# ChicyChen/LOCO-Edit

Measured on AMD Instinct MI355X. Metric: edit-directions/sec (top-5 PMP-Jacobian SVD @256^2) + vT cos-sim vs ref, higher is better.
Workload: dtype bf16x3 (split-bf16 MFMA operands, fp32 accumulate + fp32 storage); 1 GPU; CelebA-HQ DDPM 256x256 top-5 local basis (l_eye-sized mask, L=2400), t=0.6T, 12 power iterations, one GPU; multi_gpu_form=single, probes_total=5, probes_per_gpu=5, kept=5, n_iter=12, mask_L=2400, weights=synthetic seed 0, streams=2

## Files before the change

### include/loco_hip_diag.h

```cpp
#ifndef LOCO_HIP_DIAG_H
#define LOCO_HIP_DIAG_H
#include "loco_hip.h"
#ifdef __cplusplus
extern "C" {
#endif

int  loco_bench_conv(loco_ctx* ctx, int32_t cin, int32_t cout, int32_t H, int32_t W, int32_t B, int32_t mode,
                     int32_t taps, int32_t tile, int32_t iters, float* ms_avg, void* stream);

typedef struct loco_conv_desc {
    int32_t struct_size;
    int32_t Cin, Cout, Hin, Win, B, taps;
    int32_t stride, upsample, zins, mode, cpg;
    int32_t transposed, accumulate, in_arena, pad;
    int32_t Cin2, cot_cpg;
    float   res_scale;
    int32_t st_cpg;
    const float *weight, *bias;
    const float *in, *bias2, *res;
    const float *prim, *sc, *sh, *mr, *gamma, *tst, *tc;
    const float *in2, *w2, *bias2nd;
    const float *cot_d, *cot_prim, *cot_sc, *cot_sh, *cot_mr, *cot_tc;
    float* out;
    const float *st_prim, *st_mr;
// ... 59 lines not shown
    int32_t op, kind, act, B, C, T, H, W, n, k, accumulate, cos_first;
    float   eps, scale, t, cv, ce;
    float   f[5];
    int32_t pad_;
    int64_t count, split, in_bs, out_bs, aux_bs, st_bs;
    const float *x, *y, *stats, *gamma, *beta, *base;
    const float *freq, *w0, *b0, *w1, *b1, *add, *add_in;
    const float *src[4];
    const uint8_t *mask, *mask2;
    float *out, *out2, *t_dev;
} loco_pointwise_desc;
int  loco_debug_pointwise(loco_ctx* ctx, const loco_pointwise_desc* desc, void* stream);

int64_t loco_debug_tensor(loco_ctx* ctx, const char* name, float* dst, int64_t cap, void* stream);

#ifdef __cplusplus
}
#endif
#endif
```

### loco-edit_amd/csrc/conv_bf16_kernel.h

```cpp
#pragma once
#include "kernels.h"
#include <cstdlib>
#include <type_traits>

namespace loco {


typedef float f32x16 __attribute__((ext_vector_type(16)));
typedef float f32x4 __attribute__((ext_vector_type(4)));
typedef f32x4 f32x4_u __attribute__((aligned(4)));
typedef float f32x2 __attribute__((ext_vector_type(2)));
typedef f32x2 f32x2_u __attribute__((aligned(4)));
typedef __bf16 bf16x8 __attribute__((ext_vector_type(8)));
typedef _Float16 f16x8 __attribute__((ext_vector_type(8)));
typedef short s16x8 __attribute__((ext_vector_type(8)));

enum : int { PR_BF16X3 = 0, PR_F16 = 1 };

constexpr int BKC = 16;
constexpr bool LIVE_MASK = true;
constexpr bool EARLY_W = true;
constexpr int NDUMMY = 8;

__device__ __forceinline__ float sigmoidf2_(float y) { return __builtin_amdgcn_rcpf(1.0f + __expf(-y)); }
// ... 507 lines not shown
        }
        tile_id = __builtin_amdgcn_readfirstlane(tile_id);
        cot_id = __builtin_amdgcn_readfirstlane(cot_id);
        zid = __builtin_amdgcn_readfirstlane(zid);
    }
    int ty0_, tx0_;
    idivmod_small(tile_id, tiles_x, ty0_, tx0_);
    const int oy0 = __builtin_amdgcn_readfirstlane(ty0_ * TH);
    const int ox0 = __builtin_amdgcn_readfirstlane(tx0_ * TW);
    const int co0 = cot_id * MT;
    int zb_, zs_;
    idivmod_small(zid, a.nsplit, zb_, zs_);
    const int b = __builtin_amdgcn_readfirstlane(zb_);
    const int split = __builtin_amdgcn_readfirstlane(zs_);

    if constexpr (XPF && PHASE != 2 && EARLY_W) {
        const int nchunks_ = (a.Cin + BKC - 1) / BKC;
        const int cps_ = __builtin_amdgcn_readfirstlane((nchunks_ + a.nsplit - 1) / a.nsplit);
        const int cbeg_ = split * cps_;
        const int cend_ = (cbeg_ + cps_ < nchunks_) ? cbeg_ + cps_ : nchunks_;
        if (cend_ > cbeg_) {
            typedef __attribute__((address_space(3))) unsigned char lds_u8_;
            typedef const __attribute__((address_space(1))) unsigned char glb_u8_;
            const int wpitch_ = (a.Cout + 31) & ~31;
            const unsigned char* wbase0 = reinterpret_cast<const unsigned char*>(a.wb) +
                                          (unsigned)(cbeg_ * TAPS) * ((unsigned)wpitch_ * (unsigned)RB);
#pragma unroll
            for (int st_ = 0; st_ < 2; ++st_)
#pragma unroll
                for (int i = 0; i < NWV; ++i) {
// ... 837 lines not shown
```

### loco-edit_amd/csrc/conv_plan.hip

```cpp
#include "kernels.h"
#include <cstdio>
#include <cstdlib>

namespace loco {

constexpr int BKC = 16;
constexpr int BKF = 8;

static const int kMT[6] = {128, 128, 32, 64, 128, 128}, kNT[6] = {128, 64, 128, 64, 256, 256};

static int env_int(const char* name, int dflt) {
    const char* e = getenv(name);
    return e ? atoi(e) : dflt;
}
static int pick_tile(int Cout, int HW) {
    if (HW >= 128) return Cout > 32 ? 0 : 2;
    return Cout > 64 ? 1 : 3;
}

static int conv_pick_nsplit(int Cin, int Cout, int Hout, int Wout, int B) {
    const int t = pick_tile(Cout, Hout * Wout);
    long blocks = (long)((Hout * Wout) / kNT[t]) * ((Cout + kMT[t] - 1) / kMT[t]) * B;
    int nchunks = (Cin + BKF - 1) / BKF;
    if (blocks >= 384 || nchunks < 8) return 1;
// ... 14 lines not shown
    return t;
}

constexpr int kTile0MaxHW = 65536;

static int bf16_tile_of(const ConvArgs& a, int tile_override = -1) {
    int tile = conv_bf16_pick_tile(a.Cout, a.Hout * a.Wout, a.B, tile_override);
    if (tile == 4) tile = 5;
    if (tile == 5 && a.taps == 1 && !a.gemm && a.B >= 2 && a.Hout * a.Wout <= kTile0MaxHW) return 0;
    if (a.stride == 2 && tile == 5) tile = 0;
    return tile;
}
static int tile_for(const ConvArgs& a, int prec, int tile_override) {
    return prec ? bf16_tile_of(a, tile_override) : pick_tile(a.Cout, a.Hout * a.Wout);
}
static int conv_bf16_tile_pixels(const ConvArgs& a) { return a.poly == 1 ? 512 : a.gemm ? 256 : kNT[a.tile]; }
int conv_bf16_tile_couts(const ConvArgs& a) { return a.gemm ? 64 * a.gemm_tm : kMT[a.tile]; }

static bool conv_poly_ok(const ConvEnv& e, const ConvArgs& a, int taps) {
    static const bool on = env_int("LOCO_POLYPHASE", 1) != 0;
    if (!on || e.prec < 1 || taps != 9 || a.mode != CM_NONE || !(a.upsample || a.zins) || a.stride != 1) return false;
    if (!(e.prec == 2 ? a.wph : a.wpb) || !a.in_padded || a.res || a.Cin2 > 0 || a.cot_d) return false;
    if (a.upsample ? a.pad != 1 : (a.pad != 1 && a.pad != 2)) return false;
    if ((a.Cin % BKC) != 0 || (a.Cout % 128) != 0 || a.B < 2) return false;
    if (a.Hin * a.Win < 4096 || a.Win < 32 || (a.Win % 32) != 0 || (a.Hin % 8) != 0) return false;
    return a.Hout == 2 * a.Hin && a.Wout == 2 * a.Win;
}
static bool conv_poly_in_ok(const ConvEnv& e, const ConvArgs& a, int taps) {
    static const bool on = env_int("LOCO_POLYPHASE", 1) != 0;
    if (!on || e.prec < 1 || taps != 9 || a.mode != CM_NONE || !a.pool2 || a.upsample || a.zins || a.stride != 1 || a.pad != 1) return false;
    if (!(e.prec == 2 ? a.wqh : a.wqb) || a.res || a.bias2 || a.Cin2 > 0 || a.cot_d) return false;
// ... 295 lines not shown
```

### loco-edit_amd/csrc/engine.hip

```cpp
#include <hip/hip_runtime.h>

#include <algorithm>
#include <array>
#include <cmath>
#include <cstdio>
#include <cstdlib>
#include <cstring>
#include <map>
#include <memory>
#include <thread>
#include <atomic>
#include <string>
#include <vector>

#include "../../include/loco_hip.h"
#ifdef LOCO_DIAG
#include "../../include/loco_hip_diag.h"
#endif
#include "kernels.h"
#include "program.h"
#ifdef LOCO_DIAG
#include "conv_plan_text.h"
#endif

// ... 111 lines not shown
    bool has_tcond = false;
    float2* sxcache = nullptr;
    int prec = 0;
    std::vector<float*> owned;
    size_t bytes = 0;

    bool primal_ok = false;
    float p_cv = 0.f, p_ce = 0.f;
    int tap = 0;
    long n_ws = 0;
    uint8_t* mask = nullptr;
    bool has_mask = false;
    uint8_t* mask2 = nullptr;
    bool has_mask2 = false;
    int mask2_from = 0;
    int* mask_idx = nullptr;
    int* mask_L_dev = nullptr;
    long mask_L = 0;
    hipStream_t mask_stream = nullptr;
    int primal_B = 0;
    hipEvent_t ev0 = nullptr, ev1 = nullptr;
    int n_streams = 1;
    hipStream_t st2 = nullptr;
    hipStream_t st2_user = nullptr;
    hipEvent_t ev_fork = nullptr, ev_join = nullptr;
    double* red2 = nullptr;
    struct FwdGraph { hipGraph_t graph = nullptr; hipGraphExec_t exec = nullptr; int calls = 0; };
    std::map<int, FwdGraph> fwd_graphs;
    bool graph_on = false;
    bool gemm_lowp = true;
// ... 445 lines not shown
    const NormP& n = *rq.n;
    const long SB = c->prog->stats_per_sample;
    const int G = c->cfg.gn_groups;
    if (rq.kind == ST_FWD) {
        NS s = nstats(c, rq.stats + (long)s0 * SB, n);
        launch_gn_stats(x, xbs, B, n.C, HW, G, eps_of(c, n), n.gamma, n.beta, s.mr, s.sc, s.sh, SB, c->red, st, rq.ss_scale,
                        rq.ss_shift);
    } else {
        NS sp = nstats(c, c->statsP, n);
        NS stt = nstats(c, rq.stats + (long)s0 * SB, n);
        launch_gn_tstats(x, xbs, rq.prim, 0, B, n.C, HW, G, sp.sc, sp.sh, sp.mr, 0, 0, rq.kind == ST_TAN ? 0 : 1, stt.tst,
                         stt.tc, SB, c->red, st, c->cfg.act);
    }
}

bool run_conv(loco_ctx* c, const ConvArgs& a0, int taps, hipStream_t st, const StatReq* rq = nullptr,
              const ConvArgs* second = nullptr) {
    const size_t span = (size_t)c->cfg.max_batch * c->prog->per_sample;
    auto padded = [&](const float* p) { return (p >= c->arenaP && p < c->arenaP + span) || (p >= c->arenaT && p < c->arenaT + span); };
    ConvArgs a = a0, sc;
    a.act = c->cfg.act;
    if (a.mode == CM_GN_SILU && c->cfg.act == ACT_GELU) a.mode = CM_GN_GELU;
    a.in_padded = padded(a.in);
    if (second) { sc = *second; sc.in_padded = padded(sc.in); }
    ConvEnv e;
    e.prec = c->prec; e.chip_share = c->chip_share; e.lanes = c->lanes_active; e.lane_s0 = c->lane_s0;
    e.partial = c->partial; e.partial_floats = c->partial_floats; e.stpart = c->stpart; e.stpart_floats = c->stpart_floats;
    e.fuse_stats = c->fuse_stats; e.fuse_lin = c->fuse_lin; e.deep1 = c->deep1; e.max_batch = c->cfg.max_batch;
    StatAsk q;
    if (rq) {
        q.kind = rq->kind; q.norm = rq->n != nullptr; q.prim = rq->prim; q.keep = rq->keep; q.keep_floats = rq->keep_floats;
        if (rq->n && rq->n->sx_off >= 0 && c->sxcache) q.sx = c->sxcache + rq->n->sx_off;
// ... 8 lines not shown
    const int HWo = a.Hout * a.Wout, Gn = c->cfg.gn_groups;
    const long SBs = c->prog->stats_per_sample;
    auto timed = [&](const char* name, double flops, const ConvArgs& y, auto&& launch) {
        loco_ctx::ProfRec r;
        if (c->prof_on) {
            r.name = name; r.flops = flops;
            r.cin = y.Cin; r.cout = y.Cout; r.h = y.Hout; r.b = y.B; r.ns = y.nsplit; r.mode = y.mode; r.taps = taps;
            r.e0 = c->next_event(); r.e1 = c->next_event();
            (void)hipEventRecord(r.e0, st);
        }
        launch();
        if (c->prof_on) { (void)hipEventRecord(r.e1, st); c->prof.push_back(r); }
    };
    for (int li = 0; li < p.nl; ++li) {
        const ConvLaunch& l = p.l[li];
        const ConvArgs& x = l.args;
        double flops = 2.0 * (x.Cin * taps + x.Cin2) * x.Cout * (double)x.Hout * x.Wout * x.B;
        if (x.zins) flops *= 0.25;
        if (x.poly == 2) flops *= 4.0;
        timed(c->prof_on ? conv_variant_name(x, taps, c->prec) : nullptr, flops, x, [&] {
            if (c->prec == 1) launch_conv_bf16x3(x, taps, st);
            else if (c->prec == 2) launch_conv_f16(x, taps, st);
            else launch_conv(x, taps, st);
        });
        if (x.nsplit > 1) {
            timed("conv_splitk_reduce", 0.0, x, [&] {
                if (l.stats != SR_SPLITK) { launch_conv_splitk_reduce(x, st); return; }
                const NormP& n = *rq->n;
                NS sp = nstats(c, c->statsP, n);
                NS so = nstats(c, rq->stats + (long)l.s0 * SBs, n);
                launch_conv_splitk_reduce_stats(x, rq->kind, Gn, eps_of(c, n), n.gamma, n.beta, so.mr, so.sc, so.sh, SBs, rq->ss_scale,
// ... 690 lines not shown
                if (op.kind == OP_DOWN) { a.stride = 2; a.pad = op.sym_down ? 1 : 0; } else { a.upsample = 1; }
                a.out = TT(op.out); a.out_bs = PS; a.Cout = to.C; a.Hout = to.H; a.Wout = to.W; a.B = B;
                const StatReq rq = next_tan(op.out);
                run_conv(c, a, 9, st, &rq);
                break;
            }
            case OP_OUT: {
                const Tens& ti = c->tens[op.in];
                if (!op.n1.ready) tangent_stats(c, op.n1, TT(op.in), PS, TP(op.in), ti.H * ti.W, B, st);
                op.n1.ready = false;
                ConvArgs a; conv_defaults(a);
                a.in = TT(op.in); a.in_bs = PS; a.Cin = ti.C; a.Hin = ti.H; a.Win = ti.W;
                setw(a, op.conv, false);
                set_tan(c, a, op.n1, TP(op.in));
                a.out = TT(op.out); a.out_bs = PS; a.Cout = to.C; a.Hout = to.H; a.Wout = to.W; a.B = B;
                run_conv(c, a, 9, st);
                break;
            }
        }
    }
    return 0;
}

void cot_stats(loco_ctx* c, const NormP& n, const float* d, long dbs, const float* x, int HW, int B, int kind,
               hipStream_t st) {
    NS sp = nstats(c, c->statsP, n);
    NS stt = nstats(c, c->statsT, n);
    launch_gn_tstats(d, dbs, x, 0, B, n.C, HW, c->cfg.gn_groups, sp.sc, sp.sh, sp.mr, 0, 0, kind, stt.tst,
                     stt.tc, c->prog->stats_per_sample, c->red, st, c->cfg.act);
}

// ... 6 lines not shown
    auto TG = [&](int id) { return c->arenaT + c->tens[id].off; };
    auto GO = [&](const Op& o) -> const float* { return o.out == c->prog->eps_t ? ge : TG(o.out); };
    auto GOS = [&](const Op& o) -> long { return o.out == c->prog->eps_t ? (long)c->prog->n_out : PS; };
    clear_ready(c);
    for (int oi = op_hi >= 0 ? op_hi : (int)c->ops.size() - 1; oi >= op_lo; --oi) {
        Op& op = c->ops[oi];
        const Tens& to = c->tens[op.out];
        const int HW = to.H * to.W;
        switch (op.kind) {
            case OP_OUT: {
                const Tens& ti = c->tens[op.in];
                ConvArgs a; conv_defaults(a);
                a.in = GO(op); a.in_bs = GOS(op); a.Cin = to.C; a.Hin = to.H; a.Win = to.W;
                setw(a, op.conv, true);
                a.out = TG(op.a1); a.out_bs = PS; a.Cout = ti.C; a.Hout = ti.H; a.Wout = ti.W; a.B = B;
                {
                    const StatReq rq = req_lin(c, ST_COT, &op.n1, TP(op.in));
                    run_conv(c, a, 9, st, &rq);
                    op.n1.ready = false;
                }
                NS sp = nstats(c, c->statsP, op.n1);
                NS stt = nstats(c, c->statsT, op.n1);
                launch_gn_apply(2, TG(op.a1), PS, TP(op.in), 0, nullptr, 0, TG(op.in), PS, 0, B, ti.C, ti.H * ti.W, G,
                                sp.sc, sp.sh, sp.mr, 0, 0, stt.tst, c->prog->stats_per_sample, st, cfg.act);
                break;
            }
            case OP_UP: {
                const Tens& ti = c->tens[op.in];
                ConvArgs a; conv_defaults(a);
                a.in = TG(op.out); a.in_bs = PS; a.Cin = to.C; a.Hin = to.H; a.Win = to.W;
                setw(a, op.conv, true);
                a.pool2 = 1; a.pool_tmp = TG(op.up); a.pool_tmp_bs = PS;
                a.out = TG(op.in); a.out_bs = PS; a.Cout = ti.C; a.Hout = ti.H; a.Wout = ti.W; a.B = B;
                run_conv(c, a, 9, st);
                break;
            }
            case OP_DOWN: {
                const Tens& ti = c->tens[op.in];
                ConvArgs a; conv_defaults(a);
// ... 270 lines not shown
    if (dalloc(c, &c->kry[0], KRY_STATE) || dalloc(c, &c->kry[1], KRY_STATE)) return -1;
    if (dalloc(c, &c->alphas, 256) || dalloc(c, &c->cond_add, (size_t)cfg->ch * 4)) return -1;
    if (dalloc(c, &c->cond_in, (size_t)cfg->ch)) return -1;
    {
        float2* sx0 = nullptr;
        if (dalloc(c, &sx0, (size_t)c->prog->sx_total + 64)) return -1;
        c->sxcache = sx0 + 32;
    }
    {
        const char* e = getenv("LOCO_PRECISION");
        c->prec = (e && std::string(e) == "f32") ? 0 : (e && std::string(e) == "f16") ? 2 : 1;
    }
    if (dalloc(c, &c->mask2, (size_t)c->prog->n_out)) return -1;
    if (dalloc(c, &c->mask, (size_t)c->prog->n_out) || dalloc(c, &c->mask_idx, (size_t)c->prog->n_out) ||
        dalloc(c, &c->mask_L_dev, 4)) return -1;
    HIPCHK(c, hipEventCreate(&c->ev0));
    HIPCHK(c, hipEventCreate(&c->ev1));
    {
        const char* e = getenv("LOCO_STREAMS");
        c->n_streams = (e && atoi(e) == 2) ? 2 : 1;
        HIPCHK(c, hipStreamCreateWithFlags(&c->st2, hipStreamNonBlocking));
        HIPCHK(c, hipStreamCreateWithFlags(&c->cap_st, hipStreamNonBlocking));
        const char* gl = getenv("LOCO_GEMM_LOWP");
        if (gl) c->gemm_lowp = atoi(gl) != 0;
        const char* gr = getenv("LOCO_GRAPH");
        c->graph_on = gr && atoi(gr) == 1;
        HIPCHK(c, hipEventCreateWithFlags(&c->ev_fork, hipEventDisableTiming));
        HIPCHK(c, hipEventCreateWithFlags(&c->ev_join, hipEventDisableTiming));
    }
    return 0;
// ... 254 lines not shown
                launch_gn_cache(c->arenaP + th.off, op.n2.C, th.H * th.W, op.n2.C / G, s2.sc, s2.sh, s2.mr,
                                c->sxcache + op.n2.sx_off, st, c->cfg.act);
            }
        }
    }
    if (use_et) { c->p_cv = 0.f; c->p_ce = 1.f; }
    else { c->p_cv = 1.0f / std::sqrt(at); c->p_ce = -std::sqrt(1.0f - at) / std::sqrt(at); }
    if (tap == 2) c->p_cv = 0.f;
    c->tap = tap;
    c->has_mask = (mask != nullptr);
    c->has_mask2 = false;
    c->mask_L = tap == 1 ? c->prog->n_h : c->prog->n_out;
    if (mask) {
        HIPCHK(c, hipMemcpyAsync(c->mask, mask, (size_t)c->prog->n_out, hipMemcpyDeviceToDevice, st));
        launch_mask_compact(c->mask, c->prog->n_out, c->mask_idx, c->mask_L_dev, st);
        c->mask_L = -1;
        c->mask_stream = st;
    }
    HIPCHK(c, hipGetLastError());
    c->primal_ok = true;
    return 0;
}

int loco_pmp_set_second_mask(loco_ctx* c, const uint8_t* mask2, int32_t from_row, void* stream) {
    if (!c) return -2;
    if (!c->primal_ok) { c->err = "loco_pmp_primal has not been called"; return -2; }
    if (!mask2) { c->has_mask2 = false; return 0; }
    if (!c->has_mask) { c->err = "a second mask needs a first one (loco_pmp_primal with mask)"; return -2; }
    if (from_row < 0) { c->err = "from_row must be >= 0"; return -2; }
    HIPCHK(c, hipMemcpyAsync(c->mask2, mask2, (size_t)c->prog->n_out, hipMemcpyDeviceToDevice, (hipStream_t)stream));
    c->has_mask2 = true;
    c->mask2_from = from_row;
    return 0;
}

int loco_pmp_jvp(loco_ctx* c, const float* V, int32_t k, float* U, void* stream) {
    if (!c) return -2;
    if (!c->primal_ok) { c->err = "loco_pmp_primal has not been called"; return -2; }
    hipStream_t st = (hipStream_t)stream;
    const int MB = c->cfg.max_batch;
    for (int b0 = 0; b0 < k; b0 += MB) {
        int B = (k - b0 < MB) ? k - b0 : MB;
        int rc = run_lanes(c, B, st, [&](int s0, int nb, hipStream_t ls) -> int {
            const Program& P = *c->prog;
            if (c->tap == 1) {
// ... 1206 lines not shown
        if (op.name != nm) continue;
        int id = want_h1 ? op.h1 : op.out;
        if (id < 0) return -3;
        const Tens& t = c->tens[id];
        int64_t cnt = (int64_t)t.C * t.H * t.W;
        int B = arena ? 1 : (c->primal_B > 0 ? c->primal_B : 1);
        if (cnt * B > cap) { c->err = "debug buffer too small"; return -4; }
        float* base = (arena ? c->arenaT : c->arenaP) + t.off;
        launch_copy(base, c->prog->per_sample, dst, cnt, 0, B, cnt, (hipStream_t)stream);
        return cnt * B;
    }
    c->err = "no such op: " + nm;
    return -3;
}

#endif

}
```

### loco-edit_amd/csrc/kernels.h

```cpp
#pragma once
#include <hip/hip_runtime.h>
#include <stdint.h>

namespace loco {

struct DeviceOnce { bool seen[64] = {}; };
inline bool first_on_device(DeviceOnce& f) {
    int d = 0;
    (void)hipGetDevice(&d);
    d &= 63;
    if (f.seen[d]) return false;
    f.seen[d] = true;
    return true;
}


enum ConvMode : int {
    CM_NONE = 0,
    CM_GN_SILU = 1,
    CM_GN = 2,
    CM_TAN_SILU = 3,
    CM_COT_SILU = 4,
    CM_GN_GELU = 5,
};
// ... 41 lines not shown
    int B;
    float* st_part; int st_kind;
    const float* st_x; const float2* st_sx;
    const float* in2; long in2_bs; int Cin2; int in2_padded;
    const void* wb2;
    const float* cot_d; long cot_d_bs; const float2* cot_sx; const float* cot_tc; long cot_tc_bs;
    int act;
    float res_scale;
    int gemm, gemm_tm;
    size_t partial_floats;
    int tile, pair;
    const void* wpb; const void* wph;
    int poly;
    int pool2; float* pool_tmp; long pool_tmp_bs;
    const void* wqb; const void* wqh;
};

enum PolyKind : int { POLY_UP = 0, POLY_ZINS_PAD2 = 1, POLY_ZINS_PAD1 = 2 };
inline int polyphase_vcout(int C, int a, int b, int co) { return ((a * (C / 64) + co / 64) * 2 + b) * 64 + (co % 64); }
void polyphase_fold(int kind, int nin, int nout, const float* w, long so, long si, long st, float* out);
void polyphase_fold_in(int nin, int nout, const float* w, long so, long si, long st, float* out, int noutP);

void launch_conv(const ConvArgs& a, int taps, hipStream_t st);
void launch_conv_bf16x3(const ConvArgs& a, int taps, hipStream_t st);
void launch_conv_f16(const ConvArgs& a, int taps, hipStream_t st);
void launch_conv_splitk_reduce(const ConvArgs& a, hipStream_t st);

struct ConvEnv {
    int prec = 1;
    int chip_share = 1;
    int lanes = 1, lane_s0 = 0;
// ... 29 lines not shown
struct ConvPlan {
    bool sc_first = false;
    int nl = 1;
    ConvLaunch l[2];
    bool stats_all = false;
    int keep_ntile = 0;
    bool pool_after = false; float* pool_out = nullptr; long pool_out_bs = 0; int pool_acc = 0;
    bool cot = false;
};

ConvPlan plan_conv(const ConvEnv& env, const ConvArgs& a, int taps, const StatAsk* ask, const ConvArgs* shortcut);
void conv_plan_family(ConvArgs& a, int prec);
void conv_plan_tile_pair(ConvArgs& a, int prec, int tile_override);

int conv_bf16_tile_couts(const ConvArgs& a);
const char* conv_variant_name(const ConvArgs& a, int taps, int prec);

void launch_fill_random(float* p, long count, unsigned seed, float scale, hipStream_t st);
void launch_gn_cache(const float* x, int C, int HW, int cpg, const float* sc, const float* sh, const float* mr,
                     float2* sx, hipStream_t st, int act = 0);

struct GemmArgs {
    const float* A; long sam, sak, sab;
    const float* Bm; long sbk, sbn, sbb;
    float* C; long scm, scn, scb;
    const float* bias;
    const float* colbias;
    const float* R; long srb;
    int M, N, K, batch;
    float alpha, beta;
// ... 70 lines not shown
                              const float* ss_shift, hipStream_t st);
void launch_gn_lin_fused_finalize(int kind, const float* partA, int C1, int ntA, const float* partB, int ntB, int B, int C, int HW,
                                  int G, const float* mr, float* tst, float* tc, long tst_bs, hipStream_t st);
void launch_conv_splitk_reduce_stats(const ConvArgs& a, int kind, int G, float eps, const float* gamma, const float* beta,
                                     float* mr, float* sc, float* sh, long stats_bs, const float* ss_scale,
                                     const float* ss_shift, const float* prim, const float* sc_prim, const float* sh_prim,
                                     const float* mr_prim, float* tst, float* tc, long tst_bs, double* scratch,
                                     hipStream_t st);
void launch_gn_tstats(const float* d, long d_bs, const float* x, long x_bs, int B, int C, int HW, int G,
                      const float* sc, const float* sh, const float* mr, long pbs_c, long pbs_g,
                      int kind, float* tst, float* tc, long tst_bs, double* scratch, hipStream_t st, int act = 0);
void launch_gn_apply(int kind, const float* d, long d_bs, const float* x, long x_bs,
                     const float* base, long base_bs, float* out, long out_bs, int accumulate,
                     int B, int C, int HW, int G, const float* sc, const float* sh, const float* mr,
                     long pbs_c, long pbs_g, const float* tst, long tst_bs, hipStream_t st, int act = 0,
                     float base_scale = 1.0f);

void launch_ctx_groupnorm(const float* tok, int L, int D, int G, float eps, const float* gamma, const float* beta,
                          float* out, hipStream_t st);

void launch_softmax_rows(float* S, long rows, int T, hipStream_t st, int B = 1, long bs = 0);
void launch_softmax_jac(float* dS, const float* P, long rows, int T, long p_rows, float scale, hipStream_t st,
                        int B = 1, long bs = 0);

void launch_temb(float t, int ch, int temb_ch, const float* freq, const float* w0, const float* b0,
                 const float* w1, const float* b1, float* scratch, hipStream_t st, int cos_first = 0,
                 const float* add = nullptr,
                 const float* t_ptr = nullptr,
                 int act = 0,
                 const float* add_in = nullptr);
void launch_set_scalar(float* p, float v, hipStream_t st);
// ... 57 lines not shown
constexpr int KRY_THETA = KRY_W + 64 * 64;
constexpr int KRY_G = KRY_THETA + 72;
constexpr int KRY_SIGN = KRY_G + KRYLOV_MAX_BLOCK * KRYLOV_MAX_BLOCK;
constexpr int KRY_STATE = KRY_SIGN + KRYLOV_MAX_BLOCK;
void launch_krylov_fill_t(const double* Ct, int m, int k, double* T, double* Tp, hipStream_t st);
void launch_rotate_rect(const float* Q, float* out, int k, int m, long n, const double* W, int ldw, const double* sign,
                        hipStream_t st);
void launch_krylov_resid(const double* W, int m, int k, const double* G, const double* theta, float* resid, float* stat,
                         int has_prev, hipStream_t st);
void launch_krylov_floor(double* w, int k, const double* theta, float* stat, hipStream_t st);
void launch_row_sqnorm(const float* A, int k, long n, float* s, double* scratch, hipStream_t st);
void launch_edit_axpy(const float* x, const float* v, const float* alphas_dev, int B, long n, float* out,
                      hipStream_t st);
void launch_mask_gather(const float* U, const int* idx, long L, long n, int k, float* out, hipStream_t st);
void launch_mask_compact(const uint8_t* mask, long n, int* idx, int* count, hipStream_t st);

}
```

### loco-edit_amd/csrc/misc.hip

```cpp
#include "kernels.h"

namespace loco {

typedef float f32x4_t __attribute__((ext_vector_type(4)));

__device__ __forceinline__ double wave_sum(double v) {
#pragma unroll
    for (int o = 32; o > 0; o >>= 1) v += __shfl_down(v, o, 64);
    return v;
}
__device__ __forceinline__ float wave_sumf(float v) {
#pragma unroll
    for (int o = 32; o > 0; o >>= 1) v += __shfl_down(v, o, 64);
    return v;
}
__device__ __forceinline__ float wave_maxf(float v) {
#pragma unroll
    for (int o = 32; o > 0; o >>= 1) v = fmaxf(v, __shfl_down(v, o, 64));
    return v;
}
__device__ __forceinline__ double block_sum(double v, double* sm) {
    v = wave_sum(v);
    __syncthreads();
    if ((threadIdx.x & 63) == 0) sm[threadIdx.x >> 6] = v;
// ... 501 lines not shown
    if (kind == ST_FWD) {
        hipLaunchKernelGGL(gn_finalize_kernel, dim3((G + 63) / 64, a.B), dim3(64), 0, st, scratch, ns, G, a.Cout, eps, gamma,
                           beta, mr, sc, sh, stats_bs, ss_scale, ss_shift);
    } else {
        const long BG = (long)a.B * G;
        hipLaunchKernelGGL(gn_tstats_finalize, dim3((unsigned)((BG + 255) / 256)), dim3(256), 0, st, scratch, ns, BG, G,
                           1.0 / (double)len, tst, tc, tst_bs, cpg, mr_prim, 0L, kind == ST_TAN ? 0 : 1);
    }
}

template <int KIND>
__global__ __launch_bounds__(256) void gn_apply_kernel(const float* d, long d_bs, const float* x, long x_bs,
                                                       const float* base, long base_bs, float* out, long out_bs,
                                                       int accumulate, int C, int HW, int cpg, const float* sc,
                                                       const float* sh, const float* mr, long pbs_c, long pbs_g,
                                                       const float* tst, long tbs, int act, float base_scale) {
    const int b = blockIdx.y;
    const long per = (long)C * HW;
    for (long i = ((long)blockIdx.x * 256 + threadIdx.x) * 4; i < per; i += (long)gridDim.x * 1024) {
        int c = (int)(i / HW);
        int g = c / cpg;
        float scc = sc[(long)b * pbs_c + c], shc = sh[(long)b * pbs_c + c];
        float4 xv = *reinterpret_cast<const float4*>(x + (long)b * x_bs + i);
        float xx[4] = {xv.x, xv.y, xv.z, xv.w};
        float r[4];
        if (KIND == 0) {
#pragma unroll
            for (int j = 0; j < 4; ++j) r[j] = fmaf(scc, xx[j], shc);
        } else if (KIND == 4) {
#pragma unroll
            for (int j = 0; j < 4; ++j) r[j] = act_fwd(fmaf(scc, xx[j], shc), act);
        } else {
            float mean = mr[(long)b * pbs_g + 2 * g], rstd = mr[(long)b * pbs_g + 2 * g + 1];
            float m1 = tst[(long)b * tbs + g * 2], m2 = tst[(long)b * tbs + g * 2 + 1];
            float4 dv = *reinterpret_cast<const float4*>(d + (long)b * d_bs + i);
            float dd[4] = {dv.x, dv.y, dv.z, dv.w};
            float bb[4] = {0.f, 0.f, 0.f, 0.f};
            if (KIND >= 2 && base) {
                float4 bv = *reinterpret_cast<const float4*>(base + (long)b * base_bs + i);
                bb[0] = base_scale * bv.x; bb[1] = base_scale * bv.y; bb[2] = base_scale * bv.z; bb[3] = base_scale * bv.w;
            }
            float gm = scc / rstd;
#pragma unroll
            for (int j = 0; j < 4; ++j) {
                float xh = (xx[j] - mean) * rstd;
                if (KIND == 1) r[j] = scc * (dd[j] - m1 - xh * m2);
                else if (KIND == 5) r[j] = act_der(fmaf(scc, xx[j], shc), act) * scc * (dd[j] - m1 - xh * m2);
                else if (KIND == 2) r[j] = bb[j] + rstd * (gm * act_der(fmaf(scc, xx[j], shc), act) * dd[j] - m1 - xh * m2);
                else r[j] = bb[j] + rstd * (gm * dd[j] - m1 - xh * m2);
            }
        }
        float4* o = reinterpret_cast<float4*>(out + (long)b * out_bs + i);
        if (accumulate) {
            float4 ov = *o;
            r[0] += ov.x; r[1] += ov.y; r[2] += ov.z; r[3] += ov.w;
        }
        *o = make_float4(r[0], r[1], r[2], r[3]);
    }
}

void launch_gn_apply(int kind, const float* d, long d_bs, const float* x, long x_bs, const float* base,
                     long base_bs, float* out, long out_bs, int accumulate, int B, int C, int HW, int G,
                     const float* sc, const float* sh, const float* mr, long pbs_c, long pbs_g, const float* tst,
                     long tst_bs, hipStream_t st, int act, float base_scale) {
    long per = (long)C * HW;
    int blocks = (int)((per / 4 + 255) / 256);
    if (blocks > 1024) blocks = 1024;
    dim3 grid(blocks, B);
    int cpg = C / G;
#define GA(K) hipLaunchKernelGGL(gn_apply_kernel<K>, grid, dim3(256), 0, st, d, d_bs, x, x_bs, base, base_bs, out, \
                                 out_bs, accumulate, C, HW, cpg, sc, sh, mr, pbs_c, pbs_g, tst, tst_bs, act, base_scale)
    switch (kind) {
        case 0: GA(0); break;
        case 1: GA(1); break;
        case 2: GA(2); break;
        case 4: GA(4); break;
        case 5: GA(5); break;
        default: GA(3); break;
    }
#undef GA
}

__global__ __launch_bounds__(256) void gn_cache_kernel(const float* x, int C, int HW, int cpg, const float* sc,
                                                       const float* sh, const float* mr, float2* sx, int act) {
    const long per = (long)C * HW;
    for (long i = ((long)blockIdx.x * 256 + threadIdx.x) * 4; i < per; i += (long)gridDim.x * 1024) {
// ... 413 lines not shown
```

### loco-edit_amd/csrc/solver.hip

```cpp
#include "kernels.h"

namespace loco {

constexpr int GCH = 256;

__device__ __forceinline__ double wsum(double v) {
#pragma unroll
    for (int o = 32; o > 0; o >>= 1) v += __shfl_down(v, o, 64);
    return v;
}

__global__ __launch_bounds__(256) void cross_gram_partial(const float* A, int k1, const float* B, int k2, long n,
                                                          double* part, const double* gate) {
    extern __shared__ float sm[];
    if (gate && *gate == 0.0) return;
    float* As = sm;
    float* Bs = sm + (long)k1 * (GCH + 1);
    const long c0 = (long)blockIdx.x * GCH;
    for (int e = threadIdx.x; e < k1 * GCH; e += 256) {
        int i = e / GCH, c = e % GCH;
        As[i * (GCH + 1) + c] = (c0 + c < n) ? A[(long)i * n + c0 + c] : 0.f;
    }
    if (B != A) {
        for (int e = threadIdx.x; e < k2 * GCH; e += 256) {
// ... 589 lines not shown
        if (lane >= o) inc += v;
    }
    if (lane == 63) wtot[wv] = inc;
    __syncthreads();
    int base = 0;
    for (int w = 0; w < wv; ++w) base += wtot[w];
    int pos = base + inc - cnt;
    for (long i = lo; i < hi; ++i)
        if (mask[i]) idx[pos++] = (int)i;
    if (t == 1023) *count = base + inc;
}
void launch_mask_compact(const uint8_t* mask, long n, int* idx, int* count, hipStream_t st) {
    hipLaunchKernelGGL(mask_compact_kernel, dim3(1), dim3(1024), 0, st, mask, n, idx, count);
}

}
```

### loco-edit_amd/hip.py

```python
from __future__ import annotations

import ctypes as C
import os
from typing import Dict, Optional

import numpy as np
import torch

from .config import UNetConfig

_LIB_PATH = os.environ.get("LOCO_HIP_LIB") or os.path.join(os.path.dirname(os.path.abspath(__file__)), "libloco_hip.so")
_lib = None

DIAG_SYMBOLS = ["loco_bench_conv", "loco_debug_conv", "loco_debug_attn", "loco_debug_norm", "loco_debug_gemm", "loco_debug_pointwise",
                "loco_debug_tensor"]

SYMBOLS = [
    "loco_version", "loco_device_count", "loco_create", "loco_fork", "loco_destroy", "loco_last_error",
    "loco_load_param", "loco_params_missing", "loco_unet_forward", "loco_ddim_step", "loco_sched_step",
    "loco_pmp_primal", "loco_pmp_set_second_mask", "loco_pmp_jvp", "loco_pmp_vjp", "loco_orthonormalize", "loco_qr_rows",
    "loco_convergence", "loco_convergence_rows", "loco_krylov_extend", "loco_krylov_ritz", "loco_krylov_left", "loco_null_project", "loco_edit_axpy", "loco_mask_gather", "loco_mask_count",
    "loco_unet_flops", "loco_workspace_bytes", "loco_clock_stamp", "loco_set_side_stream", "loco_timer_start", "loco_timer_stop",
    "loco_profile_enable", "loco_profile_report", "loco_set_precision", "loco_get_precision", "loco_set_streams", "loco_set_chip_share",
    "loco_set_cond", "loco_set_context", "loco_lincomb", "loco_masked_axpby", "loco_latent_sample",
    "loco_text_create", "loco_text_load_param", "loco_text_params_missing", "loco_text_encode", "loco_text_last_error",
    "loco_text_destroy", "loco_t5_create", "loco_text_encode_masked",
    "loco_diffedit_mask", "loco_cfg_masked_step", "loco_set_time_cond", "loco_lcm_step",
    "loco_h_dims", "loco_unet_get_h", "loco_unet_forward_dh", "loco_pmp_primal_tap",
    "loco_sam_create", "loco_sam_load_param", "loco_sam_params_missing", "loco_sam_encode", "loco_sam_profile",
    "loco_sam_profile_read", "loco_sam_last_error", "loco_sam_destroy",
# ... 242 lines not shown
    if hasattr(lib, "loco_quality_create"):
        lib.loco_quality_create.argtypes = [C.POINTER(LocoQualityCfg), i32, i32, C.POINTER(vp)]
        lib.loco_quality_load_param.argtypes = [vp, C.c_char_p, vp, C.POINTER(i64), i32]
        lib.loco_quality_params_missing.argtypes = [vp]
        lib.loco_quality_lpips.argtypes = [vp, vp, vp, i32, i32, i32, i32, vp, vp, vp]
        lib.loco_quality_ssim.argtypes = [vp, vp, vp, i32, i32, i32, i32, C.c_double, vp, vp]
        lib.loco_quality_masked_mse.argtypes = [vp, vp, vp, vp, i32, i64, vp, vp, vp]
        lib.loco_quality_last_error.argtypes = [vp]
        lib.loco_quality_last_error.restype = C.c_char_p
        lib.loco_quality_destroy.argtypes = [vp]
        lib.loco_quality_destroy.restype = None
    if hasattr(lib, "loco_bench_conv"):
        lib.loco_bench_conv.argtypes = [vp, i32, i32, i32, i32, i32, i32, i32, i32, i32, C.POINTER(f32), vp]
        lib.loco_debug_tensor.argtypes = [vp, C.c_char_p, vp, i64, vp]
        lib.loco_debug_tensor.restype = i64
    if hasattr(lib, "loco_debug_conv"):
        lib.loco_debug_conv.argtypes = [vp, C.POINTER(LocoConvDesc), C.c_char_p, i64, vp]
    if hasattr(lib, "loco_debug_attn"):
        lib.loco_debug_attn.argtypes = [vp, C.POINTER(LocoAttnDesc), C.c_char_p, i64, vp]
    if hasattr(lib, "loco_debug_norm"):
        lib.loco_debug_norm.argtypes = [vp, C.POINTER(LocoNormDesc), vp]
    if hasattr(lib, "loco_debug_pointwise"):
        lib.loco_debug_pointwise.argtypes = [vp, C.POINTER(LocoPointwiseDesc), vp]
    if hasattr(lib, "loco_debug_gemm"):
        lib.loco_debug_gemm.argtypes = [vp, C.POINTER(LocoGemmDesc), C.c_char_p, i64, vp]
    _lib = lib
    return lib


def _ptr(t: Optional[torch.Tensor]):
# ... 656 lines not shown
        self._check(self.lib.loco_profile_report(self._ctx, buf, len(buf)), "loco_profile_report")
        out = {}
        for line in buf.value.decode().splitlines():
            name, n, ms, fl = line.rsplit(" ", 3)
            out[name] = dict(launches=int(float(n)), ms=float(ms), flops=float(fl))
        return out

    def debug_tensor(self, name: str, numel: int) -> torch.Tensor:
        self._need_diag("loco_debug_tensor")
        dst = torch.empty(numel, device=self.device, dtype=torch.float32)
        got = self.lib.loco_debug_tensor(self._ctx, name.encode(), _ptr(dst), numel, _stream())
        if got < 0:
            raise RuntimeError(f"loco_debug_tensor({name}) failed: {self.lib.loco_last_error(self._ctx).decode()}")
        return dst[:got]


class _EncoderEngine:
    _prefix = ""
    _label = ""

    def _open(self, device: Optional[torch.device]):
        self.lib = load_library()
        if not torch.cuda.is_available() or self.lib.loco_device_count() < 1:
            raise RuntimeError(f"loco_hip: no HIP device visible; the {self._label} has no CPU fallback")
        self.device = torch.device(device if device is not None else "cuda:0")
        if self.device.index is None:
            self.device = torch.device("cuda", torch.cuda.current_device())
        self._t = C.c_void_p()

    def _fn(self, name):
# ... 311 lines not shown
```

Measured before the change: 20.52 edit-directions/s.

## Skip final-conv tiles outside the mask window in tangent and cotangent passes

Builds per-tile liveness maps from the mask (and the second mask) for the eps output resolution, covering both the tile itself and its one-pixel halo. The final 3x3 conv that produces eps in the forward-tangent and cotangent passes then exits early for dead tiles, zeroing their outputs and stat partials only when later code reads them. The cotangent GroupNorm apply is told to treat dead tiles' gradients as zero instead of loading them. Since the mask covers a small region (L=2400), this is meant to cut most of that conv's work, at the cost of extra plumbing and a risk of correctness bugs when zeroed regions are read later. A debug hook for writing eps is also added.

```diff
diff --git a/include/loco_hip_diag.h b/include/loco_hip_diag.h
--- a/include/loco_hip_diag.h
+++ b/include/loco_hip_diag.h
@@ -97,6 +97,8 @@
 
 int64_t loco_debug_tensor(loco_ctx* ctx, const char* name, float* dst, int64_t cap, void* stream);
 
+int  loco_debug_poke_eps(loco_ctx* ctx, const float* src, void* stream);
+
 #ifdef __cplusplus
 }
 #endif
diff --git a/loco-edit_amd/csrc/conv_bf16_kernel.h b/loco-edit_amd/csrc/conv_bf16_kernel.h
--- a/loco-edit_amd/csrc/conv_bf16_kernel.h
+++ b/loco-edit_amd/csrc/conv_bf16_kernel.h
@@ -545,6 +545,27 @@
     const int b = __builtin_amdgcn_readfirstlane(zb_);
     const int split = __builtin_amdgcn_readfirstlane(zs_);
 
+    if constexpr (TAPS == 9 && PHASE == 0) {
+        if (a.live && !a.live[tile_id]) {
+            if ((a.live_zero & LIVE_ZERO_OUT) && co0 + MT <= a.Cout) {
+                const int twq = TW >> 2, per_co = TH * twq;
+                float* const ob = a.out + (long)b * a.out_bs + (long)co0 * a.Hout * a.Wout;
+                for (int e = tid; e < MT * per_co; e += NTHR) {
+                    int co, r, ty, q;
+                    idivmod_small(e, per_co, co, r);
+                    idivmod_small(r, twq, ty, q);
+                    *reinterpret_cast<f32x4*>(ob + (long)co * a.Hout * a.Wout + (oy0 + ty) * a.Wout + ox0 + 4 * q) = f32x4{0.f, 0.f, 0.f, 0.f};
+                }
+            }
+            if ((a.live_zero & LIVE_ZERO_PART) && a.st_part) {
+                const int ntile = (a.Hout * a.Wout) / NT;
+                float* const sp = a.st_part + (long)b * a.Cout * ntile * 2;
+                for (int r = tid; r < MT && co0 + r < a.Cout; r += NTHR)
+                    *reinterpret_cast<f32x2*>(sp + ((long)(co0 + r) * ntile + tile_id) * 2) = f32x2{0.f, 0.f};
+            }
+            return;
+        }
+    }
     if constexpr (XPF && PHASE != 2 && EARLY_W) {
         const int nchunks_ = (a.Cin + BKC - 1) / BKC;
         const int cps_ = __builtin_amdgcn_readfirstlane((nchunks_ + a.nsplit - 1) / a.nsplit);
diff --git a/loco-edit_amd/csrc/conv_plan.hip b/loco-edit_amd/csrc/conv_plan.hip
--- a/loco-edit_amd/csrc/conv_plan.hip
+++ b/loco-edit_amd/csrc/conv_plan.hip
@@ -52,7 +52,7 @@
 static int tile_for(const ConvArgs& a, int prec, int tile_override) {
     return prec ? bf16_tile_of(a, tile_override) : pick_tile(a.Cout, a.Hout * a.Wout);
 }
-static int conv_bf16_tile_pixels(const ConvArgs& a) { return a.poly == 1 ? 512 : a.gemm ? 256 : kNT[a.tile]; }
+int conv_bf16_tile_pixels(const ConvArgs& a) { return a.poly == 1 ? 512 : a.gemm ? 256 : kNT[a.tile]; }
 int conv_bf16_tile_couts(const ConvArgs& a) { return a.gemm ? 64 * a.gemm_tm : kMT[a.tile]; }
 
 static bool conv_poly_ok(const ConvEnv& e, const ConvArgs& a, int taps) {
diff --git a/loco-edit_amd/csrc/engine.hip b/loco-edit_amd/csrc/engine.hip
--- a/loco-edit_amd/csrc/engine.hip
+++ b/loco-edit_amd/csrc/engine.hip
@@ -149,6 +149,8 @@
     uint8_t* mask2 = nullptr;
     bool has_mask2 = false;
     int mask2_from = 0;
+    unsigned char* live_maps = nullptr;
+    int live_pitch = 0, end_window = 1;
     int* mask_idx = nullptr;
     int* mask_L_dev = nullptr;
     long mask_L = 0;
@@ -624,8 +626,26 @@
     }
 }
 
+struct EndWindow {
+    bool cot = false;
+    const unsigned char* gmap = nullptr; int TW = 1, TH = 1;
+};
+const unsigned char* end_window_map(const loco_ctx* c, const ConvArgs& x, int taps, bool cot, int* TW, int* TH) {
+    if (c->prec < 1 || taps != 9 || x.gemm || x.pair || x.poly || x.Cin2 > 0 || x.nsplit != 1 || x.stride != 1 || x.upsample || x.zins ||
+        x.pool2 || x.pad != 1)
+        return nullptr;
+    const Tens& te = c->tens[c->prog->eps_t];
+    if (x.Hout != te.H || x.Wout != te.W || x.Hin != te.H || x.Win != te.W) return nullptr;
+    const int NT = conv_bf16_tile_pixels(x), tw = x.Wout < 32 ? x.Wout : 32, th = NT / tw;
+    int g = NT == 64 ? 0 : NT == 128 ? 1 : NT == 256 ? 2 : -1;
+    if (g < 0 || th < 1 || th * tw != NT || (x.Wout % tw) != 0 || (x.Hout % th) != 0 || (tw & 3)) return nullptr;
+    if ((x.Hout * x.Wout) / NT > c->live_pitch || (long)x.Cout * x.Hout * x.Wout >= (1L << 31)) return nullptr;
+    *TW = tw; *TH = th;
+    return c->live_maps + (size_t)(2 * g + (cot ? 1 : 0)) * c->live_pitch;
+}
+
 bool run_conv(loco_ctx* c, const ConvArgs& a0, int taps, hipStream_t st, const StatReq* rq = nullptr,
-              const ConvArgs* second = nullptr) {
+              const ConvArgs* second = nullptr, EndWindow* ew = nullptr) {
     const size_t span = (size_t)c->cfg.max_batch * c->prog->per_sample;
     auto padded = [&](const float* p) { return (p >= c->arenaP && p < c->arenaP + span) || (p >= c->arenaT && p < c->arenaT + span); };
     ConvArgs a = a0, sc;
@@ -664,7 +684,20 @@
     };
     for (int li = 0; li < p.nl; ++li) {
         const ConvLaunch& l = p.l[li];
-        const ConvArgs& x = l.args;
+        ConvArgs x = l.args;
+        if (ew) {
+            int tw = 1, th = 1;
+            const unsigned char* m = end_window_map(c, x, taps, ew->cot, &tw, &th);
+            if (m && ew->cot) {
+                const bool unread = p.nl == 1 && !p.stats_all && l.stats != SR_ALONE && c->end_window != 2;
+                if (!unread && (x.Cout % conv_bf16_tile_couts(x)) != 0) m = nullptr;
+                else {
+                    x.live_zero = LIVE_ZERO_PART | (unread ? 0 : LIVE_ZERO_OUT);
+                    if (unread) { ew->gmap = m; ew->TW = tw; ew->TH = th; }
+                }
+            }
+            x.live = m;
+        }
         double flops = 2.0 * (x.Cin * taps + x.Cin2) * x.Cout * (double)x.Hout * x.Wout * x.B;
         if (x.zins) flops *= 0.25;
         if (x.poly == 2) flops *= 4.0;
@@ -1385,7 +1418,8 @@
                 setw(a, op.conv, false);
                 set_tan(c, a, op.n1, TP(op.in));
                 a.out = TT(op.out); a.out_bs = PS; a.Cout = to.C; a.Hout = to.H; a.Wout = to.W; a.B = B;
-                run_conv(c, a, 9, st);
+                EndWindow ew;
+                run_conv(c, a, 9, st, nullptr, nullptr, op.out == c->prog->eps_t && c->has_mask && c->end_window ? &ew : nullptr);
                 break;
             }
         }
@@ -1422,15 +1456,17 @@
                 a.in = GO(op); a.in_bs = GOS(op); a.Cin = to.C; a.Hin = to.H; a.Win = to.W;
                 setw(a, op.conv, true);
                 a.out = TG(op.a1); a.out_bs = PS; a.Cout = ti.C; a.Hout = ti.H; a.Wout = ti.W; a.B = B;
+                EndWindow ew;
+                ew.cot = true;
                 {
                     const StatReq rq = req_lin(c, ST_COT, &op.n1, TP(op.in));
-                    run_conv(c, a, 9, st, &rq);
+                    run_conv(c, a, 9, st, &rq, nullptr, op.out == c->prog->eps_t && ge && c->has_mask && c->end_window ? &ew : nullptr);
                     op.n1.ready = false;
                 }
                 NS sp = nstats(c, c->statsP, op.n1);
                 NS stt = nstats(c, c->statsT, op.n1);
                 launch_gn_apply(2, TG(op.a1), PS, TP(op.in), 0, nullptr, 0, TG(op.in), PS, 0, B, ti.C, ti.H * ti.W, G,
-                                sp.sc, sp.sh, sp.mr, 0, 0, stt.tst, c->prog->stats_per_sample, st, cfg.act);
+                                sp.sc, sp.sh, sp.mr, 0, 0, stt.tst, c->prog->stats_per_sample, st, cfg.act, 1.0f, ew.gmap, ti.W, ew.TW, ew.TH);
                 break;
             }
             case OP_UP: {
@@ -1731,6 +1767,14 @@
     if (dalloc(c, &c->mask2, (size_t)c->prog->n_out)) return -1;
     if (dalloc(c, &c->mask, (size_t)c->prog->n_out) || dalloc(c, &c->mask_idx, (size_t)c->prog->n_out) ||
         dalloc(c, &c->mask_L_dev, 4)) return -1;
+    {
+        const char* e = getenv("LOCO_END_WINDOW");
+        c->end_window = e ? atoi(e) : 1;
+        const Tens& te = c->tens[c->prog->eps_t];
+        if ((long)te.C * te.H * te.W != (long)c->prog->n_out) c->end_window = 0;
+        c->live_pitch = (te.H * te.W) / 64 + 16;
+        if (dalloc(c, &c->live_maps, (size_t)6 * c->live_pitch)) return -1;
+    }
     HIPCHK(c, hipEventCreate(&c->ev0));
     HIPCHK(c, hipEventCreate(&c->ev1));
     {
@@ -2015,6 +2059,10 @@
     if (mask) {
         HIPCHK(c, hipMemcpyAsync(c->mask, mask, (size_t)c->prog->n_out, hipMemcpyDeviceToDevice, st));
         launch_mask_compact(c->mask, c->prog->n_out, c->mask_idx, c->mask_L_dev, st);
+        if (c->end_window) {
+            const Tens& te = c->tens[c->prog->eps_t];
+            launch_mask_tile_live(c->mask, te.C, te.H, te.W, c->live_maps, c->live_pitch, 0, st);
+        }
         c->mask_L = -1;
         c->mask_stream = st;
     }
@@ -2030,6 +2078,10 @@
     if (!c->has_mask) { c->err = "a second mask needs a first one (loco_pmp_primal with mask)"; return -2; }
     if (from_row < 0) { c->err = "from_row must be >= 0"; return -2; }
     HIPCHK(c, hipMemcpyAsync(c->mask2, mask2, (size_t)c->prog->n_out, hipMemcpyDeviceToDevice, (hipStream_t)stream));
+    if (c->end_window) {
+        const Tens& te = c->tens[c->prog->eps_t];
+        launch_mask_tile_live(c->mask2, te.C, te.H, te.W, c->live_maps, c->live_pitch, 1, (hipStream_t)stream);
+    }
     c->has_mask2 = true;
     c->mask2_from = from_row;
     return 0;
@@ -3266,6 +3318,14 @@
     return -3;
 }
 
+int loco_debug_poke_eps(loco_ctx* c, const float* src, void* stream) {
+    if (!c || !src) return -2;
+    const Tens& t = c->tens[c->prog->eps_t];
+    launch_copy(src, 0, c->arenaT + t.off, c->prog->per_sample, 0, c->cfg.max_batch, (long)t.C * t.H * t.W, (hipStream_t)stream);
+    HIPCHK(c, hipGetLastError());
+    return 0;
+}
+
 #endif
 
 }
diff --git a/loco-edit_amd/csrc/kernels.h b/loco-edit_amd/csrc/kernels.h
--- a/loco-edit_amd/csrc/kernels.h
+++ b/loco-edit_amd/csrc/kernels.h
@@ -79,7 +79,9 @@
     int poly;
     int pool2; float* pool_tmp; long pool_tmp_bs;
     const void* wqb; const void* wqh;
-};
+    const unsigned char* live; int live_zero;
+};
+enum : int { LIVE_ZERO_PART = 1, LIVE_ZERO_OUT = 2 };
 
 enum PolyKind : int { POLY_UP = 0, POLY_ZINS_PAD2 = 1, POLY_ZINS_PAD1 = 2 };
 inline int polyphase_vcout(int C, int a, int b, int co) { return ((a * (C / 64) + co / 64) * 2 + b) * 64 + (co % 64); }
@@ -139,6 +141,7 @@
 void conv_plan_tile_pair(ConvArgs& a, int prec, int tile_override);
 
 int conv_bf16_tile_couts(const ConvArgs& a);
+int conv_bf16_tile_pixels(const ConvArgs& a);
 const char* conv_variant_name(const ConvArgs& a, int taps, int prec);
 
 void launch_fill_random(float* p, long count, unsigned seed, float scale, hipStream_t st);
@@ -239,7 +242,8 @@
                      const float* base, long base_bs, float* out, long out_bs, int accumulate,
                      int B, int C, int HW, int G, const float* sc, const float* sh, const float* mr,
                      long pbs_c, long pbs_g, const float* tst, long tst_bs, hipStream_t st, int act = 0,
-                     float base_scale = 1.0f);
+                     float base_scale = 1.0f,
+                     const unsigned char* live = nullptr, int lW = 1, int lTW = 1, int lTH = 1);
 
 void launch_ctx_groupnorm(const float* tok, int L, int D, int G, float eps, const float* gamma, const float* beta,
                           float* out, hipStream_t st);
@@ -327,5 +331,6 @@
                       hipStream_t st);
 void launch_mask_gather(const float* U, const int* idx, long L, long n, int k, float* out, hipStream_t st);
 void launch_mask_compact(const uint8_t* mask, long n, int* idx, int* count, hipStream_t st);
-
-}
+void launch_mask_tile_live(const uint8_t* mask, int C, int H, int W, unsigned char* maps, int pitch, int acc, hipStream_t st);
+
+}
diff --git a/loco-edit_amd/csrc/misc.hip b/loco-edit_amd/csrc/misc.hip
--- a/loco-edit_amd/csrc/misc.hip
+++ b/loco-edit_amd/csrc/misc.hip
@@ -539,7 +539,8 @@
                                                        const float* base, long base_bs, float* out, long out_bs,
                                                        int accumulate, int C, int HW, int cpg, const float* sc,
                                                        const float* sh, const float* mr, long pbs_c, long pbs_g,
-                                                       const float* tst, long tbs, int act, float base_scale) {
+                                                       const float* tst, long tbs, int act, float base_scale,
+                                                       const unsigned char* live, int lW, int lTW, int lTH) {
     const int b = blockIdx.y;
     const long per = (long)C * HW;
     for (long i = ((long)blockIdx.x * 256 + threadIdx.x) * 4; i < per; i += (long)gridDim.x * 1024) {
@@ -558,7 +559,13 @@
         } else {
             float mean = mr[(long)b * pbs_g + 2 * g], rstd = mr[(long)b * pbs_g + 2 * g + 1];
             float m1 = tst[(long)b * tbs + g * 2], m2 = tst[(long)b * tbs + g * 2 + 1];
-            float4 dv = *reinterpret_cast<const float4*>(d + (long)b * d_bs + i);
+            bool dead = false;
+            if (KIND == 2 && live) {
+                const int p = (int)(i - (long)c * HW), y = p / lW, x = p - y * lW;
+                dead = !live[(y / lTH) * (lW / lTW) + x / lTW];
+            }
+            float4 dv = make_float4(0.f, 0.f, 0.f, 0.f);
+            if (!dead) dv = *reinterpret_cast<const float4*>(d + (long)b * d_bs + i);
             float dd[4] = {dv.x, dv.y, dv.z, dv.w};
             float bb[4] = {0.f, 0.f, 0.f, 0.f};
             if (KIND >= 2 && base) {
@@ -587,14 +594,15 @@
 void launch_gn_apply(int kind, const float* d, long d_bs, const float* x, long x_bs, const float* base,
                      long base_bs, float* out, long out_bs, int accumulate, int B, int C, int HW, int G,
                      const float* sc, const float* sh, const float* mr, long pbs_c, long pbs_g, const float* tst,
-                     long tst_bs, hipStream_t st, int act, float base_scale) {
+                     long tst_bs, hipStream_t st, int act, float base_scale, const unsigned char* live, int lW, int lTW, int lTH) {
     long per = (long)C * HW;
     int blocks = (int)((per / 4 + 255) / 256);
     if (blocks > 1024) blocks = 1024;
     dim3 grid(blocks, B);
     int cpg = C / G;
 #define GA(K) hipLaunchKernelGGL(gn_apply_kernel<K>, grid, dim3(256), 0, st, d, d_bs, x, x_bs, base, base_bs, out, \
-                                 out_bs, accumulate, C, HW, cpg, sc, sh, mr, pbs_c, pbs_g, tst, tst_bs, act, base_scale)
+                                 out_bs, accumulate, C, HW, cpg, sc, sh, mr, pbs_c, pbs_g, tst, tst_bs, act, base_scale, \
+                                 kind == 2 ? live : nullptr, lW, lTW, lTH)
     switch (kind) {
         case 0: GA(0); break;
         case 1: GA(1); break;
diff --git a/loco-edit_amd/csrc/solver.hip b/loco-edit_amd/csrc/solver.hip
--- a/loco-edit_amd/csrc/solver.hip
+++ b/loco-edit_amd/csrc/solver.hip
@@ -627,4 +627,38 @@
     hipLaunchKernelGGL(mask_compact_kernel, dim3(1), dim3(1024), 0, st, mask, n, idx, count);
 }
 
-}
+__global__ __launch_bounds__(64) void mask_tile_live_kernel(const uint8_t* mask, int C, int H, int W, unsigned char* maps, int pitch,
+                                                            int acc) {
+    __shared__ int hit[2];
+    const int NT = 64 << blockIdx.y, TW = W < 32 ? W : 32, TH = NT / TW;
+    if (TH < 1 || TH * TW != NT || (W % TW) != 0 || (H % TH) != 0) return;
+    const int tiles_x = W / TW, ntile = tiles_x * (H / TH), t = blockIdx.x;
+    if (t >= ntile) return;
+    if (threadIdx.x < 2) hit[threadIdx.x] = 0;
+    __syncthreads();
+    const int y0 = (t / tiles_x) * TH, x0 = (t % tiles_x) * TW, ww = TW + 2, wsz = (TH + 2) * ww;
+    int in = 0, near = 0;
+    for (int i = threadIdx.x; i < C * wsz; i += 64) {
+        const int c = i / wsz, r = i - c * wsz, y = y0 - 1 + r / ww, x = x0 - 1 + r % ww;
+        if (y < 0 || y >= H || x < 0 || x >= W) continue;
+        if (mask[((long)c * H + y) * W + x]) {
+            near = 1;
+            if (y >= y0 && y < y0 + TH && x >= x0 && x < x0 + TW) in = 1;
+        }
+    }
+    if (in) atomicOr(&hit[0], 1);
+    if (near) atomicOr(&hit[1], 1);
+    __syncthreads();
+    if (threadIdx.x < 2) {
+        unsigned char* m = maps + (long)(2 * blockIdx.y + threadIdx.x) * pitch + t;
+        const unsigned char v = hit[threadIdx.x] ? 1 : 0;
+        *m = acc ? (unsigned char)(*m | v) : v;
+    }
+}
+void launch_mask_tile_live(const uint8_t* mask, int C, int H, int W, unsigned char* maps, int pitch, int acc, hipStream_t st) {
+    int ntile = (H * W) / 64;
+    if (ntile < 1) ntile = 1;
+    hipLaunchKernelGGL(mask_tile_live_kernel, dim3(ntile, 3), dim3(64), 0, st, mask, C, H, W, maps, pitch, acc);
+}
+
+}
diff --git a/loco-edit_amd/hip.py b/loco-edit_amd/hip.py
--- a/loco-edit_amd/hip.py
+++ b/loco-edit_amd/hip.py
@@ -13,7 +13,7 @@
 _lib = None
 
 DIAG_SYMBOLS = ["loco_bench_conv", "loco_debug_conv", "loco_debug_attn", "loco_debug_norm", "loco_debug_gemm", "loco_debug_pointwise",
-                "loco_debug_tensor"]
+                "loco_debug_tensor", "loco_debug_poke_eps"]
 
 SYMBOLS = [
     "loco_version", "loco_device_count", "loco_create", "loco_fork", "loco_destroy", "loco_last_error",
@@ -286,6 +286,8 @@
         lib.loco_bench_conv.argtypes = [vp, i32, i32, i32, i32, i32, i32, i32, i32, i32, C.POINTER(f32), vp]
         lib.loco_debug_tensor.argtypes = [vp, C.c_char_p, vp, i64, vp]
         lib.loco_debug_tensor.restype = i64
+    if hasattr(lib, "loco_debug_poke_eps"):
+        lib.loco_debug_poke_eps.argtypes = [vp, vp, vp]
     if hasattr(lib, "loco_debug_conv"):
         lib.loco_debug_conv.argtypes = [vp, C.POINTER(LocoConvDesc), C.c_char_p, i64, vp]
     if hasattr(lib, "loco_debug_attn"):
@@ -972,6 +974,11 @@
             raise RuntimeError(f"loco_debug_tensor({name}) failed: {self.lib.loco_last_error(self._ctx).decode()}")
         return dst[:got]
 
+    def debug_poke_eps(self, src: torch.Tensor):
+        self._need_diag("loco_debug_poke_eps")
+        src = src.to(self.device, torch.float32).contiguous()
+        self._check(self.lib.loco_debug_poke_eps(self._ctx, _ptr(src), _stream()), "loco_debug_poke_eps")
+
 
 class _EncoderEngine:
     _prefix = ""
```

Result: no change. 20.65 edit-directions/s, median of 6 (+0.6%).
